# baldhat/yolov10-3D

Hardware: AMD Instinct MI355X
Metric: train_images_per_sec (higher is better)
Workload: dtype bf16

## Files before the change

### include/y3d.h

```cpp
#ifndef Y3D_H
#define Y3D_H
#include <stdint.h>

#ifdef __cplusplus
extern "C" {
#endif

enum { Y3D_F32 = 0, Y3D_BF16 = 1 };
enum { Y3D_OK = 0, Y3D_ERR_INVALID = -1, Y3D_ERR_HIP = -2 };

const char* y3d_last_error(void);
int y3d_abi_version(void);
int y3d_device_info(char* name, int name_len, int* compute_units, int* lds_bytes, int* clock_khz);

int y3d_pack_weight_fwd(int dtype, const float* w_oihw, void* out, int Cout, int Cin_g, int Cin_g_pad, int kh, int kw, void* stream);
int y3d_pack_weight_dgrad(int dtype, const float* w_oihw, void* out, int Cout, int Cin_g, int groups, int kh, int kw, void* stream);
int y3d_mt_pack_weights(int dtype, const int64_t* desc, const int* chunk_tensor, const int* chunk_off, int nchunks, int chunk, void* stream);
int y3d_mt_fp8w_quantize(const int64_t* desc, const int* row_begin, int ntensors, int nrows, void* stream);
int y3d_fp8w_dequantize(const uint8_t* codes, const float* scale, float* w, int rows, int K, void* stream);
int y3d_fp8_quantize_act(const void* x, int64_t xsw, int64_t M, int C, uint8_t* q, uint8_t* s, void* stream);
int y3d_fp8_pack_weight_fwd(const uint8_t* codes, const float* scale, int rows, int Cg, uint8_t* wq, uint8_t* ws, void* stream);
int y3d_conv3x3_fp8_ok(int B, int H, int W, int Cin, int Cout, int groups);
int y3d_conv3x3_fp8_stat_rows(int B, int H, int W);
int y3d_fp8_scale_pitch(int C);
// ... 2 lines not shown
int y3d_conv_kpad(int dtype, int k_total);
int y3d_conv_stat_blocks(int B, int Ho, int Wo);
int y3d_conv2d_stat_rows(int dtype, int B, int H, int W, int Cin, int Cout, int groups, int kh, int kw, int stride, int pad);
int y3d_conv2d_fwd(int dtype, const void* x, int64_t xsb, int64_t xsh, int64_t xsw, int B, int H, int W, int Cin,
                   const void* w_packed, const float* bias, void* y, int64_t ysw, int Ho, int Wo, int Cout, int groups,
                   int kh, int kw, int stride, int pad, float* stat_partials, void* stream);
int y3d_conv2d_fwd_affine(int dtype, const void* x, int64_t xsb, int64_t xsh, int64_t xsw, int B, int H, int W, int Cin,
                          const void* w_packed, const float* scale, const float* shift, int act, void* y, int64_t ysw, int Ho, int Wo,
                          int Cout, int groups, int kh, int kw, int stride, int pad, void* stream);
int y3d_conv2d_fwd_affine_res_ok(int dtype, int B, int H, int W, int Cin, int Cout, int groups, int kh, int kw, int stride, int pad);
int y3d_conv2d_fwd_affine_res(int dtype, const void* x, int64_t xsb, int64_t xsh, int64_t xsw, int B, int H, int W, int Cin,
                              const void* w_packed, const float* scale, const float* shift, int act, const void* res, int64_t rsw, void* y,
                              int64_t ysw, int Ho, int Wo, int Cout, int groups, int kh, int kw, int stride, int pad, void* stream);
int y3d_conv2d_bwd_data(int dtype, const void* dy, int64_t dsb, int64_t dsh, int64_t dsw, int B, int Ho, int Wo, int Cout,
                        const void* w_packed_dgrad, void* dx, int64_t xsw, int H, int W, int Cin, int groups, int kh, int kw,
                        int stride, int pad, void* stream);
int y3d_conv2d_wgrad_splits(int dtype, int B, int Ho, int Wo, int Cout, int Cin_g, int groups, int kh, int kw);
int y3d_conv2d_wgrad_plan(int dtype, int B, int H, int W, int Cin, int Cout, int groups, int kh, int kw, int stride, int pad);
int y3d_set_tile_kernels(int enable);
int y3d_set_stream1x1(int enable);
int y3d_get_stream1x1(void);
int y3d_get_tile_kernels(void);
int y3d_set_bn_wide_slabs(int enable);
int y3d_conv2d_bwd_weight(int dtype, const void* x, int64_t xsb, int64_t xsh, int64_t xsw, int B, int H, int W, int Cin,
                          int Cin_real, const void* dy, int64_t dsw, int Ho, int Wo, int Cout, int groups, int kh, int kw,
                          int stride, int pad, float* slab, int nsplit, float* grad_oihw, int accumulate, void* stream);

int y3d_dw_blocks(int64_t M);
int y3d_dw_wgrad_blocks(int64_t M);
int y3d_dw_pack_weight(const float* w_oihw, float* out_taps_c, int C, int kh, int kw, void* stream);
int y3d_dwconv2d_fwd(int dtype, const void* x, int64_t xsb, int64_t xsh, int64_t xsw, int B, int H, int W, int C,
                     const float* w_packed, void* y, int64_t ysw, int Ho, int Wo, int kh, int kw, int stride, int pad,
                     float* stat_partials, void* stream);
int y3d_dwconv2d_fwd_affine(int dtype, const void* x, int64_t xsb, int64_t xsh, int64_t xsw, int B, int H, int W, int C,
                            const float* w_packed, const float* scale, const float* shift, int act, int res_mode, const void* res, int64_t rsw,
                            void* z, int64_t zsw, int Ho, int Wo, int kh, int kw, int stride, int pad, void* stream);
int y3d_dwconv2d_bwd_data(int dtype, const void* dy, int64_t dsb, int64_t dsh, int64_t dsw, int B, int Ho, int Wo, int C,
                          const float* w_packed, void* dx, int64_t xsw, int H, int W, int kh, int kw, int stride, int pad,
                          void* stream);
int y3d_dwconv2d_bwd_weight(int dtype, const void* x, int64_t xsb, int64_t xsh, int64_t xsw, int B, int H, int W, int C,
                            const void* dy, int64_t dsw, int Ho, int Wo, int kh, int kw, int stride, int pad, float* slab,
                            float* grad_oihw, int accumulate, void* stream);

int y3d_bn_finalize(const float* partials, int nblk, int C, int64_t count, const float* gamma, const float* beta, float eps,
                    float momentum, float* running_mean, float* running_var, float* mean, float* invstd, float* scale,
                    float* shift, void* stream);
// ... 138 lines not shown
```

### yolov10-3d_amd/_lib.py

```python
from __future__ import annotations

import ctypes
import os
import re

_HERE = os.path.dirname(os.path.abspath(__file__))
LIB_PATH = os.path.join(_HERE, "liby3d_hip.so")
HEADER = os.path.join(os.path.dirname(_HERE), "include", "y3d.h")

F32, BF16 = 0, 1

_CT = {"int": ctypes.c_int, "int64_t": ctypes.c_int64, "float": ctypes.c_float, "double": ctypes.c_double}


class Y3DError(RuntimeError):
    pass


def parse_header(path: str = HEADER):
    src = open(path).read()
    src = re.sub(r"/\*.*?\*/", " ", src, flags=re.S)
    protos = {}
    for m in re.finditer(r"(const\s+char\s*\*|int)\s+(y3d_\w+)\s*\(([^;{]*?)\)\s*;", src, flags=re.S):
        ret, name, args = m.group(1), m.group(2), m.group(3).strip()
        argtypes = []
        if args and args != "void":
            for a in args.split(","):
                a = a.strip()
                if "*" in a:
                    argtypes.append(ctypes.c_void_p)
                else:
                    toks = a.split()
                    t = toks[1] if toks[0] == "const" else toks[0]
                    argtypes.append(_CT[t])
        protos[name] = (ctypes.c_char_p if "char" in ret else ctypes.c_int, argtypes)
    return protos


_PLAIN_INT = {"abi_version", "conv_kpad", "conv_stat_blocks", "conv2d_stat_rows", "conv2d_wgrad_splits", "conv2d_wgrad_plan", "set_tile_kernels", "set_stream1x1", "set_bn_wide_slabs", "get_stream1x1", "get_tile_kernels", "dw_blocks", "dw_wgrad_blocks", "bn_bwd_blocks", "proj_blocks", "proj_group_blocks", "proj_group_bn_bwd_blocks", "proj_group_bwd_weight_bn_mfma_blocks", "tal3d_scratch_floats", "v10_postprocess_scratch_floats", "conv2d_fwd_affine_res_ok", "stem_conv_train_rows", "conv3x3_fp8_ok", "conv3x3_fp8_stat_rows", "fp8_scale_pitch"}


class _Lib:
    def __init__(self):
        if not os.path.exists(LIB_PATH):
            raise Y3DError(
                f"{LIB_PATH} not found: build it with `python yolov10-3d_amd/csrc/build.py` "
                "(or __graft_entry__.build()). There is no CPU / PyTorch fallback for the HIP path.")
        self._dll = ctypes.CDLL(LIB_PATH)
        self.protos = parse_header()
        for name, (ret, argtypes) in self.protos.items():
            fn = getattr(self._dll, name)
            fn.restype = ret
            fn.argtypes = argtypes

    def last_error(self) -> str:
        return (self._dll.y3d_last_error() or b"").decode()

    def __getattr__(self, name):
        if name.startswith("_"):
            raise AttributeError(name)
        fn = getattr(self._dll, "y3d_" + name)
        ret = self.protos["y3d_" + name][0]
        if ret is not ctypes.c_int or name in _PLAIN_INT:
            setattr(self, name, fn)
            return fn

        def call(*a):
            rc = fn(*a)
            if rc != 0:
                raise Y3DError(f"y3d_{name} failed ({rc}): {self.last_error()}")
            return rc

        setattr(self, name, call)
        return call


# ... 9 lines not shown
```

### yolov10-3d_amd/csrc/conv3x3_flat.hip

```cpp
#include "common.h"

namespace {


struct WFP {
  const bf16_t* x;
  const bf16_t* w;
  bf16_t* y;
  float* part;
  const float* scale;
  const float* shift;
  int act;
  long xsb, xsh, xsw, ysw;
  int B, H, W;
  int Cg, Cn, G;
  int Ktot;
  int ntf, ntc;
  int flip;
  unsigned xbytes, wbytes;
  int HP, WP, IMG;
  int HPIX;
  float inv_img, inv_wp;
};

template <int N> __device__ __forceinline__ void wvm() { asm volatile("s_waitcnt vmcnt(%0)" ::"n"(N) : "memory"); }

__device__ __forceinline__ void wvm_n(int n) {
  switch (n) {
    case 0: wvm<0>(); break; case 1: wvm<1>(); break; case 2: wvm<2>(); break; case 3: wvm<3>(); break;
    case 4: wvm<4>(); break; case 5: wvm<5>(); break; case 6: wvm<6>(); break; case 7: wvm<7>(); break;
    case 8: wvm<8>(); break; case 9: wvm<9>(); break; case 10: wvm<10>(); break; case 11: wvm<11>(); break;
    case 12: wvm<12>(); break; case 13: wvm<13>(); break; case 14: wvm<14>(); break; case 15: wvm<15>(); break;
    case 16: wvm<16>(); break; case 17: wvm<17>(); break; case 18: wvm<18>(); break; case 19: wvm<19>(); break;
    case 20: wvm<20>(); break; case 21: wvm<21>(); break; case 22: wvm<22>(); break; case 23: wvm<23>(); break;
    case 24: wvm<24>(); break; case 25: wvm<25>(); break; case 26: wvm<26>(); break; case 27: wvm<27>(); break;
    case 28: wvm<28>(); break;
    default: wvm<0>(); break;
  }
}

__device__ __forceinline__ bf16x8_t ldf(const char* p) { return __builtin_bit_cast(bf16x8_t, *(const uint4*)p); }
__device__ __forceinline__ void lgk0() { asm volatile("s_waitcnt lgkmcnt(0)" ::: "memory"); }

template <int NHB, int EPI, bool HROLE>
__device__ __forceinline__ void flat_body(const WFP& p) {
  constexpr int HD = NHB - 1;
  constexpr int RD = 4, D = 3;
  constexpr int WB = 8192;
  extern __shared__ __attribute__((aligned(16))) char smem[];
  const int HBYTES = p.HPIX * 64;
  const int NI = p.HPIX >> 4;
  const int HR = NI >> 2;
  char* sH = smem;
  char* sW = smem + NHB * HBYTES;
  float* red = (float*)(sW + RD * WB);

  const int tid = threadIdx.x, lane = tid & 63, wave = __builtin_amdgcn_readfirstlane(tid >> 6);
  const int wc = wave & 1, wp = wave >> 1;
  const int wl = wave & 3;
  const int nslab = (p.Cg + 31) >> 5;

  const int ntiles = p.G * p.ntf * p.ntc;
  int tile, tile_end, tile_step;
  {
    const int xcd = blockIdx.x & 7, slot = blockIdx.x >> 3;
    tile_step = gridDim.x >> 3;
    const int lo = (int)((long)ntiles * xcd / 8);
    tile_end = (int)((long)ntiles * (xcd + 1) / 8);
    tile = lo + slot;
  }
  if (tile >= tile_end) return;

  struct TileC { int g, f0, c0, tf, live; };
  auto decode = [&](int t, bool live) {
    TileC c;
    int tc = t % p.ntc; t /= p.ntc;
    c.tf = t % p.ntf; c.g = t / p.ntf;
    c.f0 = c.tf * 512; c.c0 = tc * 128; c.live = live;
    return c;
  };

  constexpr unsigned OOB = 0xfffffff0u;
  const __amdgpu_buffer_rsrc_t rx = __builtin_amdgcn_make_buffer_rsrc((void*)p.x, 0, (int)p.xbytes, 0x00020000);
  const __amdgpu_buffer_rsrc_t rw = __builtin_amdgcn_make_buffer_rsrc((void*)p.w, 0, (int)p.wbytes, 0x00020000);
  const int xsw2 = (int)p.xsw * 2, xsh2 = (int)p.xsh * 2, xsb2 = (int)p.xsb * 2;
  const int lj0 = lane >> 2;
  const int pc0 = ((lane & 3) << 4) ^ ((lj0 & 4) << 3);
  const int a64 = 64 / p.WP, c64 = 64 - a64 * p.WP;
  int hb = 0, hy = 0, hx = 0;
  auto issue_h = [&](const TileC& c, int slab, int bufo, int rd) {
    if (rd == 0) {
      int lj = lj0;
      asm volatile("" : "+v"(lj));
      const int fs = c.f0 - (p.WP + 1) + 16 * wl + lj + p.IMG;
      int q = (int)((float)fs * p.inv_img);
      int r = fs - q * p.IMG;
      if (r < 0) { r += p.IMG; --q; }
      if (r >= p.IMG) { r -= p.IMG; ++q; }
      int y = (int)((float)r * p.inv_wp);
      int x = r - y * p.WP;
      if (x < 0) { x += p.WP; --y; }
// ... 9 lines not shown
    const unsigned off = (unsigned)(hb * xsb2 + (hy - 1) * xsh2 + __mul24(hx - 1, xsw2) + (c.g * p.Cg + slab * 32) * 2 + pc0);
    char* dst = sH + bufo + (rd * 4 + wl) * 1024;
    __builtin_amdgcn_raw_ptr_buffer_load_lds(rx, (__attribute__((address_space(3))) void*)dst, 16, ok ? off : OOB, 0, 0, 0);
  };
  const int ltid = tid & 255;
  int wrel0, wrel1, wch;
  {
    const int n0 = ltid >> 2, s = ltid & 3;
    wch = (s ^ (((n0 >> 4) & 1) << 1)) << 3;
    wrel0 = (n0 * p.Ktot + wch) * 2;
    wrel1 = ((n0 + 64) * p.Ktot + wch) * 2;
  }
  auto issue_w = [&](const TileC& c, int slab, int tap, int slot, int rd) {
    const unsigned base = (unsigned)((c.g * p.Cn + c.c0) * p.Ktot + (p.flip ? 8 - tap : tap) * p.Cg + slab * 32) * 2u;
    const int n = rd * 64 + (ltid >> 2);
    const bool ok = (c.live != 0) & (c.c0 + n < p.Cn) & (wch < p.Cg - slab * 32);
    __builtin_amdgcn_raw_ptr_buffer_load_lds(rw, (__attribute__((address_space(3))) void*)(sW + slot * WB + (rd * 256 + wl * 64) * 16), 16,
                                             ok ? base + (unsigned)(rd ? wrel1 : wrel0) : OOB, 0, 0, 0);
  };

  const int lp = lane & 15, lq = lane >> 4;
  const int arow = wc * 64 + (lp >> 2) * 8 + (lp & 3);
  const int ao = arow * 64 + ((lq ^ (((arow >> 4) & 1) << 1)) << 4);
  const int pb0 = wp * 128 + lp;
  bf16x8_t fa[4], fb[4];
  int bo;
  auto set_tap = [&](int tap) {
    const int r = tap / 3, q = tap - r * 3;
    const int pb = pb0 + r * p.WP + q;
    bo = (pb << 6) + ((lq ^ ((pb >> 1) & 2)) << 4);
  };
  auto load_b = [&](int bufo, int half) {
    const char* hbp = sH + bufo + bo;
#pragma unroll
    for (int i = 0; i < 4; ++i) fb[i] = ldf(hbp + (half * 4 + i) * 1024);
  };
  auto load_a = [&](int slot) {
#pragma unroll
    for (int ct = 0; ct < 4; ++ct) fa[ct] = ldf(sW + slot * WB + ao + (ct >> 1) * 2048 + (ct & 1) * 256);
  };

  TileC cur = decode(tile, true);
  TileC nx = decode(tile + tile_step < tile_end ? tile + tile_step : tile, tile + tile_step < tile_end);
  if (HROLE) {
#pragma unroll 1
    for (int h = 0; h < HD; ++h)
#pragma unroll 1
      for (int rd = 0; rd < HR; ++rd) issue_h(cur, h, h * HBYTES, rd);
    wvm_n((HD - 1) * HR);
  } else {
#pragma unroll
    for (int t = 0; t < D; ++t) { issue_w(cur, 0, t, t, 0); issue_w(cur, 0, t, t, 1); }
    wvm<2 * (D - 1)>();
  }
  __builtin_amdgcn_s_barrier();

  int gs = 0;
  int ho_cur = 0, ho_nxt = HBYTES, ho_tgt = (NHB - 1) * HBYTES;
  int tolerate = 0;
#pragma unroll 1
  for (; tile < tile_end; tile += tile_step) {
    f32x4_t acc[4][8];
#pragma unroll
    for (int a = 0; a < 4; ++a)
#pragma unroll
      for (int c = 0; c < 8; ++c) acc[a][c] = (f32x4_t){0.f, 0.f, 0.f, 0.f};

    if (!HROLE) __builtin_amdgcn_s_barrier();

#pragma unroll 1
    for (int k = 0; k < nslab; ++k, ++gs) {
      const bool last = k == nslab - 1;
      const int kr = gs & 3;
      const int hb_cur = ho_cur, hb_nxt = ho_nxt, hb_tgt = ho_tgt;
      if (NHB == 3) { ho_cur = hb_nxt; ho_nxt = hb_tgt; ho_tgt = hb_cur; } else { ho_cur = hb_nxt; ho_nxt = hb_cur; ho_tgt = hb_cur; }
      const bool hin = k + HD < nslab;
      const int hs = hin ? k + HD : k + HD - nslab;
      const TileC htile = hin ? cur : nx;
      const TileC wtile = last ? nx : cur;
      const int wslab = last ? 0 : k + 1;
#pragma unroll
      for (int t = 0; t < 9; ++t) {
        const int t2 = t + D;
        set_tap(t);
        load_a((kr + t) & 3);
        load_b(hb_cur, 0);
        __builtin_amdgcn_sched_barrier(0);
        if (HROLE) {
          if (2 * t < HR) issue_h(htile, hs, hb_tgt, 2 * t);
        } else {
          if (t2 < 9) issue_w(cur, k, t2, (kr + t2) & 3, 0); else issue_w(wtile, wslab, t2 - 9, (kr + t2) & 3, 0);
        }
        __builtin_amdgcn_sched_barrier(0);
        lgk0();
        __builtin_amdgcn_sched_barrier(0);
        __builtin_amdgcn_s_barrier();
        __builtin_amdgcn_s_setprio(1);
#pragma unroll
        for (int ct = 0; ct < 4; ++ct)
#pragma unroll
          for (int i = 0; i < 4; ++i) acc[ct][i] = __builtin_amdgcn_mfma_f32_16x16x32_bf16(fa[ct], fb[i], acc[ct][i], 0, 0, 0);
        __builtin_amdgcn_s_setprio(0);
        __builtin_amdgcn_sched_barrier(0);
        __builtin_amdgcn_s_barrier();
        load_b(hb_cur, 1);
        __builtin_amdgcn_sched_barrier(0);
        if (HROLE) {
          if (2 * t + 1 < HR) issue_h(htile, hs, hb_tgt, 2 * t + 1);
          if (t == 8) { if (NHB == 3) wvm_n(HR); else wvm<0>(); }
        } else {
          if (t2 < 9) issue_w(cur, k, t2, (kr + t2) & 3, 1); else issue_w(wtile, wslab, t2 - 9, (kr + t2) & 3, 1);
          if (k == 0 && t < 2) wvm_n(2 * (D - 1) + tolerate);
          else wvm<2 * (D - 1)>();
        }
        __builtin_amdgcn_sched_barrier(0);
        lgk0();
        __builtin_amdgcn_sched_barrier(0);
        __builtin_amdgcn_s_barrier();
        __builtin_amdgcn_s_setprio(1);
#pragma unroll
        for (int ct = 0; ct < 4; ++ct)
#pragma unroll
          for (int i = 0; i < 4; ++i) acc[ct][4 + i] = __builtin_amdgcn_mfma_f32_16x16x32_bf16(fa[ct], fb[i], acc[ct][4 + i], 0, 0, 0);
        __builtin_amdgcn_s_setprio(0);
        __builtin_amdgcn_sched_barrier(0);
        __builtin_amdgcn_s_barrier();
      }
    }
    if (HROLE) __builtin_amdgcn_s_barrier();

    int el = ltid;
    asm volatile("" : "+v"(el));
    const int e_lp = el & 15, e_lq = (el >> 4) & 3;
    const int e_tid = (HROLE ? 0 : 256) + el;
    const int cl0 = wc * 64 + e_lq * 8;
    const int a16 = 16 / p.WP, c16 = 16 - a16 * p.WP;
    int eb, ey, ex;
    {
      const int f = cur.f0 + wp * 128 + e_lp;
      int q = (int)((float)f * p.inv_img);
      int r = f - q * p.IMG;
      if (r < 0) { r += p.IMG; --q; }
      if (r >= p.IMG) { r -= p.IMG; ++q; }
      int y = (int)((float)r * p.inv_wp);
      int x = r - y * p.WP;
      if (x < 0) { x += p.WP; --y; }
      if (x >= p.WP) { x -= p.WP; ++y; }
      eb = q; ey = y; ex = x;
    }
    bool cok[2];
    typedef float f2_t __attribute__((ext_vector_type(2)));
    typedef __bf16 b2_t __attribute__((ext_vector_type(2)));
    f2_t s2[2][4], q2[2][4];
    float sv[2][8], hv[2][8];
#pragma unroll
    for (int h = 0; h < 2; ++h) {
      cok[h] = cur.c0 + cl0 + h * 32 < p.Cn;
#pragma unroll
      for (int i = 0; i < 4; ++i) { s2[h][i] = (f2_t){0.f, 0.f}; q2[h][i] = (f2_t){0.f, 0.f}; }
      if (EPI == 1) {
#pragma unroll
        for (int i = 0; i < 8; ++i) {
          sv[h][i] = cok[h] ? p.scale[cur.g * p.Cn + cur.c0 + cl0 + h * 32 + i] : 1.f;
          hv[h][i] = cok[h] ? p.shift[cur.g * p.Cn + cur.c0 + cl0 + h * 32 + i] : 0.f;
        }
      }
    }
    int issued = 0;
#pragma unroll
    for (int pt = 0; pt < 8; ++pt) {
      const bool pok = ((unsigned)eb < (unsigned)p.B) & ((unsigned)(ey - 1) < (unsigned)p.H) & ((unsigned)(ex - 1) < (unsigned)p.W);
      const unsigned keep = pok ? 0xffffffffu : 0u;
      bf16_t* dst = p.y + (((long)eb * p.H + (ey - 1)) * p.W + (ex - 1)) * p.ysw + (long)cur.g * p.Cn + cur.c0 + cl0;
#pragma unroll
      for (int h = 0; h < 2; ++h) {
        if (EPI == 0) {
          unsigned pk[4];
#pragma unroll
          for (int c2 = 0; c2 < 2; ++c2)
#pragma unroll
            for (int jj = 0; jj < 2; ++jj) {
              const f2_t a = {acc[2 * h + c2][pt][2 * jj], acc[2 * h + c2][pt][2 * jj + 1]};
              const unsigned u = __builtin_bit_cast(unsigned, __builtin_convertvector(a, b2_t)) & keep;
              pk[c2 * 2 + jj] = u;
              const f2_t r = {__uint_as_float(u << 16), __uint_as_float(u & 0xffff0000u)};
              s2[h][c2 * 2 + jj] += r;
              q2[h][c2 * 2 + jj] = __builtin_elementwise_fma(r, r, q2[h][c2 * 2 + jj]);
            }
          if (pok && cok[h]) *(uint4*)(dst + h * 32) = make_uint4(pk[0], pk[1], pk[2], pk[3]);
        } else {
          float v[8];
#pragma unroll
          for (int c2 = 0; c2 < 2; ++c2)
// ... 27 lines not shown
      lgk0();
      __builtin_amdgcn_s_barrier();
      if (e_tid < 128) {
        const int ch = e_tid;
        if (cur.c0 + ch < p.Cn) {
          float s = 0.f, q = 0.f;
#pragma unroll
          for (int w = 0; w < 4; ++w) { s += red[(w * 128 + ch) * 2]; q += red[(w * 128 + ch) * 2 + 1]; }
          float* dst = p.part + ((long)cur.tf * (p.G * p.Cn) + cur.g * p.Cn + cur.c0 + ch) * 2;
          *(float2*)dst = make_float2(s, q);
        }
      }
    }
    tolerate = __builtin_amdgcn_readfirstlane(issued);
    cur = nx;
    {
      const int t2 = tile + 2 * tile_step;
      nx = decode(t2 < tile_end ? t2 : tile, t2 < tile_end);
    }
  }
  wvm<0>();
}

template <int NHB, int EPI>
__global__ __launch_bounds__(512, 1) void conv3x3_flat_kernel(WFP p) {
  if (__builtin_amdgcn_readfirstlane(threadIdx.x >> 6) < 4) flat_body<NHB, EPI, true>(p);
  else flat_body<NHB, EPI, false>(p);
}

int flat_cu_count() {
  static int n = 0;
  if (!n) {
    int dev = 0;
    hipDeviceProp_t pr;
    if (hipGetDevice(&dev) == hipSuccess && hipGetDeviceProperties(&pr, dev) == hipSuccess) n = pr.multiProcessorCount;
    if (n <= 0) n = 256;
  }
  return n;
}

template <int NHB, int EPI>
int launch_flat(const WFP& p, hipStream_t st) {
  size_t sm = (size_t)NHB * p.HPIX * 64 + 4 * 8192 + 4 * 128 * 2 * 4;
  static bool attr_set = false;
  if (!attr_set) {
    (void)hipFuncSetAttribute((const void*)conv3x3_flat_kernel<NHB, EPI>, hipFuncAttributeMaxDynamicSharedMemorySize, 160 * 1024);
    attr_set = true;
  }
  long ntiles = (long)p.G * p.ntf * p.ntc;
  long nwg = (long)flat_cu_count() / 8 * 8;
  if (nwg < 8) nwg = 8;
  while (nwg > 8 && nwg / 8 > (ntiles + 7) / 8) nwg -= 8;
  hipLaunchKernelGGL((conv3x3_flat_kernel<NHB, EPI>), dim3((unsigned)nwg), dim3(512), sm, st, p);
  Y3D_LAUNCH_CHECK();
  return Y3D_OK;
}

}

static int flat_hpix(int W) { return (512 + 2 * (W + 3) + 63) / 64 * 64; }

int y3d_conv3x3_flat_tiles(int B, int H, int W) { return cdiv((long)B * (H + 2) * (W + 2), 512); }

int y3d_conv3x3_flat_ok(int B, int H, int W, int Cg, int Cn, int G) {
  if (Cg % 8 != 0 || Cg < 40 || Cn % 16 != 0 || W < 8 || W > 126 || H < 8) return 0;
  if ((size_t)2 * flat_hpix(W) * 64 + 4 * 8192 + 4096 > 160 * 1024) return 0;
  if ((long)B * (H + 2) * (W + 2) >= (1L << 23)) return 0;
  return 1;
}

int y3d_conv3x3_flat_launch(const void* x, long xsb, long xsh, long xsw, int B, int H, int W, int Cg, int Cn, int G, const void* w, int Ktot, void* y,
                            long ysw, float* part, int flip, const float* scale, const float* shift, int act, void* stream) {
  WFP p;
  p.x = (const bf16_t*)x; p.w = (const bf16_t*)w; p.y = (bf16_t*)y; p.part = part; p.scale = scale; p.shift = shift; p.act = act;
  p.xsb = xsb; p.xsh = xsh; p.xsw = xsw; p.ysw = ysw;
  p.B = B; p.H = H; p.W = W; p.Cg = Cg; p.Cn = Cn; p.G = G; p.Ktot = Ktot;
  p.HP = H + 2; p.WP = W + 2; p.IMG = p.HP * p.WP; p.HPIX = flat_hpix(W);
  p.inv_img = 1.0f / (float)p.IMG; p.inv_wp = 1.0f / (float)p.WP;
  p.ntf = y3d_conv3x3_flat_tiles(B, H, W); p.ntc = cdiv(Cn, 128); p.flip = flip;
  const unsigned long xb = ((unsigned long)(B - 1) * xsb + (unsigned long)(H - 1) * xsh + (unsigned long)(W - 1) * xsw + (unsigned long)G * Cg) * 2;
  const unsigned long wb = (unsigned long)G * Cn * Ktot * 2;
  Y3D_CHECK(xb < 0xfffffff0ul && wb < 0xfffffff0ul, "conv3x3_flat: operand larger than 4 GB");
  Y3D_CHECK(2 * xsw < (1L << 23) && Ktot < (1 << 22), "conv3x3_flat: pixel stride beyond the 24-bit address multiply");
  Y3D_CHECK(y3d_conv3x3_flat_ok(B, H, W, Cg, Cn, G), "conv3x3_flat: geometry not served");
  p.xbytes = (unsigned)xb; p.wbytes = (unsigned)wb;
  hipStream_t st = (hipStream_t)stream;
  const bool three = (size_t)3 * p.HPIX * 64 + 4 * 8192 + 4096 <= 160 * 1024;
  if (three) return scale ? launch_flat<3, 1>(p, st) : launch_flat<3, 0>(p, st);
  return scale ? launch_flat<2, 1>(p, st) : launch_flat<2, 0>(p, st);
}
```

### yolov10-3d_amd/csrc/conv3x3_tile.hip

```cpp
#include "common.h"
#include <cstdlib>
#include "conv_frag.h"

namespace {

__device__ uint4 y3d_zero_page[4];
#ifdef Y3D_PROBE_STAMP
__device__ unsigned long long y3d_probe_stamps[16384 * 4];
#define Y3D_STAMP(i) if (threadIdx.x == 0 && blockIdx.z * gridDim.x + blockIdx.x < 16384) y3d_probe_stamps[(blockIdx.z * gridDim.x + blockIdx.x) * 4 + (i)] = __builtin_amdgcn_s_memtime()
#else
#define Y3D_STAMP(i)
#endif

struct C3P {
  const void* x;
  const void* w;
  void* y;
  float* part;
  const float* scale;
  const float* shift;
  int act;
  long xsb, xsh, xsw, ysw;
  int B, H, W;
  int Cg, Cn, G;
// ... 242 lines not shown
  constexpr int RD = TH == 16 ? 4 : 2;
  size_t sm = 2 * (size_t)HCH * 16 + (size_t)RD * 16384;
  static bool attr_set = false;
  if (!attr_set) {
    (void)hipFuncSetAttribute((const void*)conv3x3_tile_kernel<T, TH, EPI>, hipFuncAttributeMaxDynamicSharedMemorySize, (int)sm);
    attr_set = true;
  }
  dim3 grid(p.B * p.nty * p.ntx * p.ntc, 1, p.G);
  hipLaunchKernelGGL((conv3x3_tile_kernel<T, TH, EPI>), grid, dim3(NT), sm, st, p);
  Y3D_LAUNCH_CHECK();
  return Y3D_OK;
}

template <typename T, int TH>
int launch_tile_epi(const C3P& p, hipStream_t st) {
  return p.scale ? launch_tile<T, TH, 1>(p, st) : launch_tile<T, TH, 0>(p, st);
}

}

int y3d_conv3x3_wide3_launch(int th, const void* x, long xsb, long xsh, long xsw, int B, int H, int W, int Cg, int Cn, int G, const void* w,
                             int Ktot, void* y, long ysw, float* part, int flip, const float* scale, const float* shift, int act, void* stream);

int y3d_conv3x3_flat_ok(int B, int H, int W, int Cg, int Cn, int G);
int y3d_conv3x3_flat_tiles(int B, int H, int W);
int y3d_conv3x3_flat_launch(const void* x, long xsb, long xsh, long xsw, int B, int H, int W, int Cg, int Cn, int G, const void* w, int Ktot, void* y,
                            long ysw, float* part, int flip, const float* scale, const float* shift, int act, void* stream);

static int v2_max_tiles() { return 129; }

int y3d_tile_height(int dtype, int B, int H, int W, int Cg, int Cn, int G, int kh, int kw, int stride, int pad) {
  int cse = 32;
  if (kh != 3 || kw != 3 || stride != 1 || pad != 1) return 0;
  if (dtype == Y3D_BF16 ? (Cg % 8 != 0 || Cg < 40 || (Cg < 64 && Cg % 32 != 0 && Cn <= 64)) : (Cg % cse != 0 || Cg < 64)) return 0;
  if (Cn % 16 != 0) return 0;
  if (W < 8) return 0;
  if (dtype == Y3D_BF16 && y3d_conv3x3_flat_ok(B, H, W, Cg, Cn, G)) {
    const int thr = H % 16 == 0 ? 16 : 8;
    const long rect = (long)cdiv(B, 32 / thr) * cdiv(H, thr) * cdiv(W, 16), flat = y3d_conv3x3_flat_tiles(B, H, W);
    if (flat * 104 < rect * 100 && flat * G * cdiv(Cn, 128) >= v2_max_tiles()) return -1;
  }
  if (H % 16 == 0) return 16;
  if (H % 8 == 0) return 8;
  if (dtype == Y3D_BF16 && H > 8 && (H % 8) >= 4 && (long)G * cdiv(B, 4) * cdiv(H, 8) * cdiv(W, 16) * cdiv(Cn, 128) >= v2_max_tiles()) return 8;
  return 0;
}

int y3d_conv3x3_tile_launch(int dtype, int th, const void* x, long xsb, long xsh, long xsw, int B, int H, int W, int Cg, int Cn, int G,
                            const void* w, int Ktot, void* y, long ysw, float* part, int flip, const float* scale, const float* shift, int act,
                            void* stream) {
  C3P p;
  p.x = x; p.w = w; p.y = y; p.part = part; p.scale = scale; p.shift = shift; p.act = act;
  p.xsb = xsb; p.xsh = xsh; p.xsw = xsw; p.ysw = ysw;
  p.B = B; p.H = H; p.W = W; p.Cg = Cg; p.Cn = Cn; p.G = G; p.Ktot = Ktot;
  p.ntx = cdiv(W, 16); p.nty = cdiv(H, th); p.ntc = cdiv(Cn, 128); p.flip = flip;
  hipStream_t st = (hipStream_t)stream;
  if (th < 0) return y3d_conv3x3_flat_launch(x, xsb, xsh, xsw, B, H, W, Cg, Cn, G, w, Ktot, y, ysw, part, flip, scale, shift, act, stream);
  if (dtype == Y3D_BF16) {
    const long wide_tiles = (long)G * cdiv(B, 32 / th) * p.nty * p.ntx * p.ntc;
    if (wide_tiles < v2_max_tiles() && Cg % 64 == 0 && H % th == 0)
      return th == 16 ? launch_tile_epi<bf16_t, 16>(p, st) : launch_tile_epi<bf16_t, 8>(p, st);
    return y3d_conv3x3_wide3_launch(th, x, xsb, xsh, xsw, B, H, W, Cg, Cn, G, w, Ktot, y, ysw, part, flip, scale, shift, act, stream);
  }
  return th == 16 ? launch_tile_epi<float, 16>(p, st) : launch_tile_epi<float, 8>(p, st);
}
```

### yolov10-3d_amd/csrc/conv_gemm.hip

```cpp
#include "common.h"
#include "conv_frag.h"
#include <cstdlib>

namespace {

struct ConvP {
  const void* x;
  const void* w;
  const float* bias;
  const float* scale;
  const float* shift;
  int act;
  void* y;
  float* part;
  long xsb, xsh, xsw;
  long ysw;
  int B, Hg, Wg;
  int Hq, Wq;
  int Cg, Cn, G;
  int kh, kw, stride, pad;
  int Ktot, Kpad;
  int M;
  int ntx, nty;
};
// ... 631 lines not shown
  if (bc == 128) {
    size_t sm = 2 * (128 + 128) * 128;
    hipLaunchKernelGGL((conv_gemm_kernel<T, 128, 128, 2, 2, MODE>), dim3(p.ntx * p.nty, ny, p.G), block, sm, st, p);
  } else if (bc == 64) {
    size_t sm = 2 * (128 + 64) * 128;
    hipLaunchKernelGGL((conv_gemm_kernel<T, 128, 64, 4, 1, MODE>), dim3(p.ntx * p.nty, ny, p.G), block, sm, st, p);
  } else {
    size_t sm = 2 * (128 + 32) * 128;
    hipLaunchKernelGGL((conv_gemm_kernel<T, 128, 32, 4, 1, MODE>), dim3(p.ntx * p.nty, ny, p.G), block, sm, st, p);
  }
  Y3D_LAUNCH_CHECK();
  return Y3D_OK;
}

template <typename T, bool DGRAD>
int launch_conv(ConvP p, hipStream_t st) {
  if (DGRAD && p.kh == 3 && p.kw == 3 && p.stride == 2 && p.pad == 1 && p.Cg % TT<T>::CE == 0) return launch_conv_mode<T, 2>(p, st);
  return launch_conv_mode<T, DGRAD ? 1 : 0>(p, st);
}

}

int y3d_tile_height(int dtype, int B, int H, int W, int Cg, int Cn, int G, int kh, int kw, int stride, int pad);
int y3d_conv3x3_flat_tiles(int B, int H, int W);
int y3d_conv3x3_tile_launch(int dtype, int th, const void* x, long xsb, long xsh, long xsw, int B, int H, int W, int Cg, int Cn, int G,
                            const void* w, int Ktot, void* y, long ysw, float* part, int flip, const float* scale, const float* shift, int act,
                            void* stream);

int y3d_wgrad_tile_height(int dtype, int H, int W, int Cg, int Cn, int kh, int kw, int stride, int pad);
int y3d_wgrad_tile_splits(int th, int B, int H, int W, int Cg, int Cn, int G);
int y3d_conv3x3_wgrad_tile_launch(int th, const void* x, long xsb, long xsh, long xsw, const void* dy, long dsw, int B, int H, int W, int Cg,
                                  int Cn, int G, float* slab, int nsplit, void* stream);

int y3d_conv1x1_stream_ok(int dtype, long M, int K, int N, long xsw, int G = 1);
int y3d_conv1x1_stream_launch(const void* x, long xsw, const void* w, int Kpad, const float* bias, const float* scale, const float* shift, int act,
                              void* y, long ysw, float* part, long M, int K, int N, int G, void* stream);
int y3d_wgrad1x1_stream_ok(int dtype, long M, int Cg, int Cn, long xsw, long dsw);
int y3d_wgrad1x1_stream_launch(const void* x, long xsw, const void* dy, long dsw, long M, int Cg, int Cn, float* slab, int nsplit, int chunk_px,
                               void* stream);
int y3d_conv3x3s2_dgrad_ok(int dtype, int B, int Ho, int Wo, int H, int W, int Cout, int Cin, long dsw, long xsw);
int y3d_conv3x3s2_dgrad_launch(const void* dy, long dsw, int B, int Ho, int Wo, int Cout, const void* w_packed_dgrad, int Kpad, void* dx, long xsw,
                               int H, int W, int Cin, void* stream);
int y3d_conv3x3_small_ok(int dtype, int B, int H, int W, int Cin, int Cout, int rows);
int y3d_conv3x3_small_launch(const void* x, long xsb, long xsh, long xsw, int B, int H, int W, int Cin, int Cout, const void* w, int Ktot, void* y,
                             long ysw, float* part, int rows, int flip, const float* scale, const float* shift, int act, const void* res, long rsw,
                             void* stream);
int y3d_conv3x3_small_rows(int B, int H, int W, int Cin, int Cout);
// ... 30 lines not shown
  if (kh == 3 && kw == 3 && stride == 1 && pad == 1 && groups == 1 && y3d_wgrad3x3_small_ok(dtype, B, H, W, Cin, Cout))
    return y3d_wgrad3x3_small_splits(B, H, W);
  int th = (g_tile_kernels && groups > 0) ? y3d_wgrad_tile_height(dtype, H, W, Cin / groups, Cout / groups, kh, kw, stride, pad) : 0;
  if (th) return y3d_wgrad_tile_splits(th, B, H, W, Cin / groups, Cout / groups, groups);
  int Ho = (H + 2 * pad - kh) / stride + 1, Wo = (W + 2 * pad - kw) / stride + 1;
  if (kh == 1 && kw == 1 && stride == 1 && pad == 0 && groups == 1 && y3d_wgrad1x1_stream_ok(dtype, (long)B * H * W, Cin, Cout, Cin, Cout)) {
    const int target = 256;
    const long tiles = (long)cdiv(Cin, Cin <= 64 ? 64 : 128) * cdiv(Cout, Cout <= 64 ? 64 : 128);
    long want = target / tiles, maxs = cdiv((long)B * H * W, 4 * 64);
    if (want > maxs) want = maxs;
    return (int)(want < 1 ? 1 : want);
  }
  return y3d_conv2d_wgrad_splits(dtype, B, Ho, Wo, Cout, Cin / groups, groups, kh, kw);
}

int y3d_conv2d_stat_rows(int dtype, int B, int H, int W, int Cin, int Cout, int groups, int kh, int kw, int stride, int pad) {
  if (kh == 1 && kw == 1 && stride == 1 && pad == 0 && groups >= 1 && y3d_conv1x1_stream_ok(dtype, (long)B * H * W, Cin / groups, Cout / groups, Cin, groups))
    return y3d_conv1x1_stream_rows((long)B * H * W, Cin / groups, Cout / groups, groups);
  if (kh == 3 && kw == 3 && stride == 1 && pad == 1 && groups == 1 && y3d_conv3x3_small_ok(dtype, B, H, W, Cin, Cout, 1))
    return y3d_conv3x3_small_rows(B, H, W, Cin, Cout);
  if (kh == 3 && kw == 3 && stride == 2 && pad == 1 && groups == 1 && y3d_conv3x3_small_s2_ok(dtype, B, H, W, Cin, Cout))
    return y3d_conv3x3_small_s2_rows(B, H, W, Cin, Cout);
  int th = (g_tile_kernels && groups > 0) ? y3d_tile_height(dtype, B, H, W, Cin / groups, Cout / groups, groups, kh, kw, stride, pad) : 0;
  if (th < 0) return y3d_conv3x3_flat_tiles(B, H, W);
  if (th) return B * cdiv(H, th) * cdiv(W, 16);
  int Ho = (H + 2 * pad - kh) / stride + 1, Wo = (W + 2 * pad - kw) / stride + 1;
  return cdiv((long)B * Ho * Wo, 128);
}

int y3d_conv_kpad(int dtype, int k_total) {
  int ce = dtype == Y3D_BF16 ? 8 : 4;
  return cdiv(k_total, ce) * ce;
}

int y3d_pack_weight_fwd(int dtype, const float* w_oihw, void* out, int Cout, int Cin_g, int Cin_g_pad, int kh, int kw, void* stream) {
  int ce = dtype == Y3D_BF16 ? 8 : 4;
  Y3D_CHECK(Cin_g_pad >= Cin_g && Cin_g_pad % ce == 0, "pack_weight_fwd: Cin_g_pad=%d must be a multiple of %d", Cin_g_pad, ce);
  int taps = kh * kw, Kpad = taps * Cin_g_pad;
  long n = (long)Cout * Kpad;
  hipStream_t st = (hipStream_t)stream;
  if (dtype == Y3D_BF16)
    hipLaunchKernelGGL(pack_w_fwd_kernel<bf16_t>, dim3(cdiv(n, 256)), dim3(256), 0, st, w_oihw, (bf16_t*)out, Cout, Cin_g, Cin_g_pad, taps, Kpad);
  else
    hipLaunchKernelGGL(pack_w_fwd_kernel<float>, dim3(cdiv(n, 256)), dim3(256), 0, st, w_oihw, (float*)out, Cout, Cin_g, Cin_g_pad, taps, Kpad);
  Y3D_LAUNCH_CHECK();
  return Y3D_OK;
}
// ... 230 lines not shown
```

Measured before the change: 1425.

## Add 256-position flat conv3x3 tile variant with cost-model tiling selection

```diff
diff --git a/include/y3d.h b/include/y3d.h
--- a/include/y3d.h
+++ b/include/y3d.h
@@ -48,6 +48,8 @@
 int y3d_get_stream1x1(void);
 int y3d_get_tile_kernels(void);
 int y3d_set_bn_wide_slabs(int enable);
+int y3d_set_flat256(int mode);
+int y3d_conv3x3_tiling(int dtype, int B, int H, int W, int Cg, int Cn, int G);
 int y3d_conv2d_bwd_weight(int dtype, const void* x, int64_t xsb, int64_t xsh, int64_t xsw, int B, int H, int W, int Cin,
                           int Cin_real, const void* dy, int64_t dsw, int Ho, int Wo, int Cout, int groups, int kh, int kw,
                           int stride, int pad, float* slab, int nsplit, float* grad_oihw, int accumulate, void* stream);
diff --git a/yolov10-3d_amd/_lib.py b/yolov10-3d_amd/_lib.py
--- a/yolov10-3d_amd/_lib.py
+++ b/yolov10-3d_amd/_lib.py
@@ -37,7 +37,7 @@
     return protos
 
 
-_PLAIN_INT = {"abi_version", "conv_kpad", "conv_stat_blocks", "conv2d_stat_rows", "conv2d_wgrad_splits", "conv2d_wgrad_plan", "set_tile_kernels", "set_stream1x1", "set_bn_wide_slabs", "get_stream1x1", "get_tile_kernels", "dw_blocks", "dw_wgrad_blocks", "bn_bwd_blocks", "proj_blocks", "proj_group_blocks", "proj_group_bn_bwd_blocks", "proj_group_bwd_weight_bn_mfma_blocks", "tal3d_scratch_floats", "v10_postprocess_scratch_floats", "conv2d_fwd_affine_res_ok", "stem_conv_train_rows", "conv3x3_fp8_ok", "conv3x3_fp8_stat_rows", "fp8_scale_pitch"}
+_PLAIN_INT = {"abi_version", "conv_kpad", "conv_stat_blocks", "conv2d_stat_rows", "conv2d_wgrad_splits", "conv2d_wgrad_plan", "set_tile_kernels", "set_stream1x1", "set_bn_wide_slabs", "set_flat256", "conv3x3_tiling", "get_stream1x1", "get_tile_kernels", "dw_blocks", "dw_wgrad_blocks", "bn_bwd_blocks", "proj_blocks", "proj_group_blocks", "proj_group_bn_bwd_blocks", "proj_group_bwd_weight_bn_mfma_blocks", "tal3d_scratch_floats", "v10_postprocess_scratch_floats", "conv2d_fwd_affine_res_ok", "stem_conv_train_rows", "conv3x3_fp8_ok", "conv3x3_fp8_stat_rows", "fp8_scale_pitch"}
 
 
 class _Lib:
@@ -52,6 +52,9 @@
             fn = getattr(self._dll, name)
             fn.restype = ret
             fn.argtypes = argtypes
+        flat256 = os.environ.get("Y3D_FLAT256")
+        if flat256 in ("0", "1", "2"):
+            self._dll.y3d_set_flat256(int(flat256))
 
     def last_error(self) -> str:
         return (self._dll.y3d_last_error() or b"").decode()
diff --git a/yolov10-3d_amd/csrc/conv3x3_flat.hip b/yolov10-3d_amd/csrc/conv3x3_flat.hip
--- a/yolov10-3d_amd/csrc/conv3x3_flat.hip
+++ b/yolov10-3d_amd/csrc/conv3x3_flat.hip
@@ -42,8 +42,10 @@
 __device__ __forceinline__ bf16x8_t ldf(const char* p) { return __builtin_bit_cast(bf16x8_t, *(const uint4*)p); }
 __device__ __forceinline__ void lgk0() { asm volatile("s_waitcnt lgkmcnt(0)" ::: "memory"); }
 
-template <int NHB, int EPI, bool HROLE>
+template <int NP, int NHB, int EPI, bool HROLE>
 __device__ __forceinline__ void flat_body(const WFP& p) {
+  static_assert(NP == 512 || NP == 256, "flat tile of 512 or 256 positions");
+  constexpr int PW = NP / 4, NC = PW / 16, NH = NC / 2;
   constexpr int HD = NHB - 1;
   constexpr int RD = 4, D = 3;
   constexpr int WB = 8192;
@@ -76,7 +78,7 @@
     TileC c;
     int tc = t % p.ntc; t /= p.ntc;
     c.tf = t % p.ntf; c.g = t / p.ntf;
-    c.f0 = c.tf * 512; c.c0 = tc * 128; c.live = live;
+    c.f0 = c.tf * NP; c.c0 = tc * 128; c.live = live;
     return c;
   };
 
@@ -132,8 +134,8 @@
   const int lp = lane & 15, lq = lane >> 4;
   const int arow = wc * 64 + (lp >> 2) * 8 + (lp & 3);
   const int ao = arow * 64 + ((lq ^ (((arow >> 4) & 1) << 1)) << 4);
-  const int pb0 = wp * 128 + lp;
-  bf16x8_t fa[4], fb[4];
+  const int pb0 = wp * PW + lp;
+  bf16x8_t fa[4], fb[NH];
   int bo;
   auto set_tap = [&](int tap) {
     const int r = tap / 3, q = tap - r * 3;
@@ -143,7 +145,7 @@
   auto load_b = [&](int bufo, int half) {
     const char* hbp = sH + bufo + bo;
 #pragma unroll
-    for (int i = 0; i < 4; ++i) fb[i] = ldf(hbp + (half * 4 + i) * 1024);
+    for (int i = 0; i < NH; ++i) fb[i] = ldf(hbp + (half * NH + i) * 1024);
   };
   auto load_a = [&](int slot) {
 #pragma unroll
@@ -170,11 +172,11 @@
   int tolerate = 0;
 #pragma unroll 1
   for (; tile < tile_end; tile += tile_step) {
-    f32x4_t acc[4][8];
+    f32x4_t acc[4][NC];
 #pragma unroll
     for (int a = 0; a < 4; ++a)
 #pragma unroll
-      for (int c = 0; c < 8; ++c) acc[a][c] = (f32x4_t){0.f, 0.f, 0.f, 0.f};
+      for (int c = 0; c < NC; ++c) acc[a][c] = (f32x4_t){0.f, 0.f, 0.f, 0.f};
 
     if (!HROLE) __builtin_amdgcn_s_barrier();
 
@@ -209,7 +211,7 @@
 #pragma unroll
         for (int ct = 0; ct < 4; ++ct)
 #pragma unroll
-          for (int i = 0; i < 4; ++i) acc[ct][i] = __builtin_amdgcn_mfma_f32_16x16x32_bf16(fa[ct], fb[i], acc[ct][i], 0, 0, 0);
+          for (int i = 0; i < NH; ++i) acc[ct][i] = __builtin_amdgcn_mfma_f32_16x16x32_bf16(fa[ct], fb[i], acc[ct][i], 0, 0, 0);
         __builtin_amdgcn_s_setprio(0);
         __builtin_amdgcn_sched_barrier(0);
         __builtin_amdgcn_s_barrier();
@@ -231,7 +233,7 @@
 #pragma unroll
         for (int ct = 0; ct < 4; ++ct)
 #pragma unroll
-          for (int i = 0; i < 4; ++i) acc[ct][4 + i] = __builtin_amdgcn_mfma_f32_16x16x32_bf16(fa[ct], fb[i], acc[ct][4 + i], 0, 0, 0);
+          for (int i = 0; i < NH; ++i) acc[ct][NH + i] = __builtin_amdgcn_mfma_f32_16x16x32_bf16(fa[ct], fb[i], acc[ct][NH + i], 0, 0, 0);
         __builtin_amdgcn_s_setprio(0);
         __builtin_amdgcn_sched_barrier(0);
         __builtin_amdgcn_s_barrier();
@@ -247,7 +249,7 @@
     const int a16 = 16 / p.WP, c16 = 16 - a16 * p.WP;
     int eb, ey, ex;
     {
-      const int f = cur.f0 + wp * 128 + e_lp;
+      const int f = cur.f0 + wp * PW + e_lp;
       int q = (int)((float)f * p.inv_img);
       int r = f - q * p.IMG;
       if (r < 0) { r += p.IMG; --q; }
@@ -278,7 +280,7 @@
     }
     int issued = 0;
 #pragma unroll
-    for (int pt = 0; pt < 8; ++pt) {
+    for (int pt = 0; pt < NC; ++pt) {
       const bool pok = ((unsigned)eb < (unsigned)p.B) & ((unsigned)(ey - 1) < (unsigned)p.H) & ((unsigned)(ex - 1) < (unsigned)p.W);
       const unsigned keep = pok ? 0xffffffffu : 0u;
       bf16_t* dst = p.y + (((long)eb * p.H + (ey - 1)) * p.W + (ex - 1)) * p.ysw + (long)cur.g * p.Cn + cur.c0 + cl0;
@@ -352,10 +354,10 @@
   wvm<0>();
 }
 
-template <int NHB, int EPI>
+template <int NP, int NHB, int EPI>
 __global__ __launch_bounds__(512, 1) void conv3x3_flat_kernel(WFP p) {
-  if (__builtin_amdgcn_readfirstlane(threadIdx.x >> 6) < 4) flat_body<NHB, EPI, true>(p);
-  else flat_body<NHB, EPI, false>(p);
+  if (__builtin_amdgcn_readfirstlane(threadIdx.x >> 6) < 4) flat_body<NP, NHB, EPI, true>(p);
+  else flat_body<NP, NHB, EPI, false>(p);
 }
 
 int flat_cu_count() {
@@ -369,53 +371,58 @@
   return n;
 }
 
-template <int NHB, int EPI>
+template <int NP, int NHB, int EPI>
 int launch_flat(const WFP& p, hipStream_t st) {
   size_t sm = (size_t)NHB * p.HPIX * 64 + 4 * 8192 + 4 * 128 * 2 * 4;
   static bool attr_set = false;
   if (!attr_set) {
-    (void)hipFuncSetAttribute((const void*)conv3x3_flat_kernel<NHB, EPI>, hipFuncAttributeMaxDynamicSharedMemorySize, 160 * 1024);
+    (void)hipFuncSetAttribute((const void*)conv3x3_flat_kernel<NP, NHB, EPI>, hipFuncAttributeMaxDynamicSharedMemorySize, 160 * 1024);
     attr_set = true;
   }
   long ntiles = (long)p.G * p.ntf * p.ntc;
   long nwg = (long)flat_cu_count() / 8 * 8;
   if (nwg < 8) nwg = 8;
   while (nwg > 8 && nwg / 8 > (ntiles + 7) / 8) nwg -= 8;
-  hipLaunchKernelGGL((conv3x3_flat_kernel<NHB, EPI>), dim3((unsigned)nwg), dim3(512), sm, st, p);
+  hipLaunchKernelGGL((conv3x3_flat_kernel<NP, NHB, EPI>), dim3((unsigned)nwg), dim3(512), sm, st, p);
   Y3D_LAUNCH_CHECK();
   return Y3D_OK;
 }
 
 }
 
-static int flat_hpix(int W) { return (512 + 2 * (W + 3) + 63) / 64 * 64; }
-
-int y3d_conv3x3_flat_tiles(int B, int H, int W) { return cdiv((long)B * (H + 2) * (W + 2), 512); }
-
-int y3d_conv3x3_flat_ok(int B, int H, int W, int Cg, int Cn, int G) {
+static int flat_hpix(int W, int np) { return (np + 2 * (W + 3) + 63) / 64 * 64; }
+
+int y3d_conv3x3_flat_tiles(int B, int H, int W, int np) { return cdiv((long)B * (H + 2) * (W + 2), np); }
+
+int y3d_conv3x3_flat_ok(int B, int H, int W, int Cg, int Cn, int G, int np) {
+  if (np != 512 && np != 256) return 0;
   if (Cg % 8 != 0 || Cg < 40 || Cn % 16 != 0 || W < 8 || W > 126 || H < 8) return 0;
-  if ((size_t)2 * flat_hpix(W) * 64 + 4 * 8192 + 4096 > 160 * 1024) return 0;
+  if ((size_t)2 * flat_hpix(W, np) * 64 + 4 * 8192 + 4096 > 160 * 1024) return 0;
   if ((long)B * (H + 2) * (W + 2) >= (1L << 23)) return 0;
   return 1;
 }
 
 int y3d_conv3x3_flat_launch(const void* x, long xsb, long xsh, long xsw, int B, int H, int W, int Cg, int Cn, int G, const void* w, int Ktot, void* y,
-                            long ysw, float* part, int flip, const float* scale, const float* shift, int act, void* stream) {
+                            long ysw, float* part, int flip, const float* scale, const float* shift, int act, int np, void* stream) {
   WFP p;
   p.x = (const bf16_t*)x; p.w = (const bf16_t*)w; p.y = (bf16_t*)y; p.part = part; p.scale = scale; p.shift = shift; p.act = act;
   p.xsb = xsb; p.xsh = xsh; p.xsw = xsw; p.ysw = ysw;
   p.B = B; p.H = H; p.W = W; p.Cg = Cg; p.Cn = Cn; p.G = G; p.Ktot = Ktot;
-  p.HP = H + 2; p.WP = W + 2; p.IMG = p.HP * p.WP; p.HPIX = flat_hpix(W);
+  p.HP = H + 2; p.WP = W + 2; p.IMG = p.HP * p.WP; p.HPIX = flat_hpix(W, np);
   p.inv_img = 1.0f / (float)p.IMG; p.inv_wp = 1.0f / (float)p.WP;
-  p.ntf = y3d_conv3x3_flat_tiles(B, H, W); p.ntc = cdiv(Cn, 128); p.flip = flip;
+  p.ntf = y3d_conv3x3_flat_tiles(B, H, W, np); p.ntc = cdiv(Cn, 128); p.flip = flip;
   const unsigned long xb = ((unsigned long)(B - 1) * xsb + (unsigned long)(H - 1) * xsh + (unsigned long)(W - 1) * xsw + (unsigned long)G * Cg) * 2;
   const unsigned long wb = (unsigned long)G * Cn * Ktot * 2;
   Y3D_CHECK(xb < 0xfffffff0ul && wb < 0xfffffff0ul, "conv3x3_flat: operand larger than 4 GB");
   Y3D_CHECK(2 * xsw < (1L << 23) && Ktot < (1 << 22), "conv3x3_flat: pixel stride beyond the 24-bit address multiply");
-  Y3D_CHECK(y3d_conv3x3_flat_ok(B, H, W, Cg, Cn, G), "conv3x3_flat: geometry not served");
+  Y3D_CHECK(y3d_conv3x3_flat_ok(B, H, W, Cg, Cn, G, np), "conv3x3_flat: geometry not served (%d-position tiles)", np);
   p.xbytes = (unsigned)xb; p.wbytes = (unsigned)wb;
   hipStream_t st = (hipStream_t)stream;
   const bool three = (size_t)3 * p.HPIX * 64 + 4 * 8192 + 4096 <= 160 * 1024;
-  if (three) return scale ? launch_flat<3, 1>(p, st) : launch_flat<3, 0>(p, st);
-  return scale ? launch_flat<2, 1>(p, st) : launch_flat<2, 0>(p, st);
-}
+  if (np == 256) {
+    Y3D_CHECK(three, "conv3x3_flat: 256-position halo buffers do not fit");
+    return scale ? launch_flat<256, 3, 1>(p, st) : launch_flat<256, 3, 0>(p, st);
+  }
+  if (three) return scale ? launch_flat<512, 3, 1>(p, st) : launch_flat<512, 3, 0>(p, st);
+  return scale ? launch_flat<512, 2, 1>(p, st) : launch_flat<512, 2, 0>(p, st);
+}
diff --git a/yolov10-3d_amd/csrc/conv3x3_tile.hip b/yolov10-3d_amd/csrc/conv3x3_tile.hip
--- a/yolov10-3d_amd/csrc/conv3x3_tile.hip
+++ b/yolov10-3d_amd/csrc/conv3x3_tile.hip
@@ -288,12 +288,64 @@
 int y3d_conv3x3_wide3_launch(int th, const void* x, long xsb, long xsh, long xsw, int B, int H, int W, int Cg, int Cn, int G, const void* w,
                              int Ktot, void* y, long ysw, float* part, int flip, const float* scale, const float* shift, int act, void* stream);
 
-int y3d_conv3x3_flat_ok(int B, int H, int W, int Cg, int Cn, int G);
-int y3d_conv3x3_flat_tiles(int B, int H, int W);
+int y3d_conv3x3_flat_ok(int B, int H, int W, int Cg, int Cn, int G, int np);
+int y3d_conv3x3_flat_tiles(int B, int H, int W, int np);
 int y3d_conv3x3_flat_launch(const void* x, long xsb, long xsh, long xsw, int B, int H, int W, int Cg, int Cn, int G, const void* w, int Ktot, void* y,
-                            long ysw, float* part, int flip, const float* scale, const float* shift, int act, void* stream);
+                            long ysw, float* part, int flip, const float* scale, const float* shift, int act, int np, void* stream);
 
 static int v2_max_tiles() { return 129; }
+
+static int g_flat256 = 1;
+
+static int rect_height(int dtype, int B, int H, int W, int Cn, int G) {
+  if (H % 16 == 0) return 16;
+  if (H % 8 == 0) return 8;
+  if (dtype == Y3D_BF16 && H > 8 && (H % 8) >= 4 && (long)G * cdiv(B, 4) * cdiv(H, 8) * cdiv(W, 16) * cdiv(Cn, 128) >= v2_max_tiles()) return 8;
+  return 0;
+}
+
+static bool tile_kernel_takes(int th, int B, int H, int W, int Cg, int Cn, int G) {
+  const long wide_tiles = (long)G * cdiv(B, 32 / th) * cdiv(H, th) * cdiv(W, 16) * cdiv(Cn, 128);
+  return wide_tiles < v2_max_tiles() && Cg % 64 == 0 && H % th == 0;
+}
+
+struct TilingCost { long ns_per_k, k0; };
+static const TilingCost kCostWide = {23, 100}, kCostFlat512 = {23, 100}, kCostFlat256 = {13, 540};
+static long persistent_rounds(long tiles) { return cdiv(cdiv(tiles, 8), 32); }
+static long round_ns(const TilingCost& c, long K) { return c.ns_per_k * (K + c.k0); }
+
+static int flat_cost_pick(int round4, int B, int H, int W, int Cg, int Cn, int G) {
+  const int rect = rect_height(Y3D_BF16, B, H, W, Cn, G);
+  const long ntc = (long)G * cdiv(Cn, 128);
+  const long K = 9L * 32 * cdiv(Cg, 32);
+  long best = -1, work = 0;
+  int code = round4;
+  auto consider = [&](long c, long w, int th) {
+    if (best < 0 || c < best || (c == best && w < work)) { best = c; work = w; code = th; }
+  };
+  if (rect > 0 && !tile_kernel_takes(rect, B, H, W, Cg, Cn, G)) {
+    const long t = cdiv(B, 32 / rect) * cdiv(H, rect) * cdiv(W, 16) * ntc;
+    consider(persistent_rounds(t) * round_ns(kCostWide, K), t * 512, rect);
+  }
+  if (y3d_conv3x3_flat_ok(B, H, W, Cg, Cn, G, 512)) {
+    const long t = y3d_conv3x3_flat_tiles(B, H, W, 512) * ntc;
+    consider(persistent_rounds(t) * round_ns(kCostFlat512, K), t * 512, -1);
+  }
+  if (y3d_conv3x3_flat_ok(B, H, W, Cg, Cn, G, 256)) {
+    const long t = y3d_conv3x3_flat_tiles(B, H, W, 256) * ntc;
+    consider(persistent_rounds(t) * round_ns(kCostFlat256, K), t * 256, -2);
+  }
+  return code;
+}
+
+static int round4_height(int dtype, int B, int H, int W, int Cg, int Cn, int G) {
+  if (dtype == Y3D_BF16 && y3d_conv3x3_flat_ok(B, H, W, Cg, Cn, G, 512)) {
+    const int thr = H % 16 == 0 ? 16 : 8;
+    const long rect = (long)cdiv(B, 32 / thr) * cdiv(H, thr) * cdiv(W, 16), flat = y3d_conv3x3_flat_tiles(B, H, W, 512);
+    if (flat * 104 < rect * 100 && flat * G * cdiv(Cn, 128) >= v2_max_tiles()) return -1;
+  }
+  return rect_height(dtype, B, H, W, Cn, G);
+}
 
 int y3d_tile_height(int dtype, int B, int H, int W, int Cg, int Cn, int G, int kh, int kw, int stride, int pad) {
   int cse = 32;
@@ -301,15 +353,30 @@
   if (dtype == Y3D_BF16 ? (Cg % 8 != 0 || Cg < 40 || (Cg < 64 && Cg % 32 != 0 && Cn <= 64)) : (Cg % cse != 0 || Cg < 64)) return 0;
   if (Cn % 16 != 0) return 0;
   if (W < 8) return 0;
-  if (dtype == Y3D_BF16 && y3d_conv3x3_flat_ok(B, H, W, Cg, Cn, G)) {
-    const int thr = H % 16 == 0 ? 16 : 8;
-    const long rect = (long)cdiv(B, 32 / thr) * cdiv(H, thr) * cdiv(W, 16), flat = y3d_conv3x3_flat_tiles(B, H, W);
-    if (flat * 104 < rect * 100 && flat * G * cdiv(Cn, 128) >= v2_max_tiles()) return -1;
-  }
-  if (H % 16 == 0) return 16;
-  if (H % 8 == 0) return 8;
-  if (dtype == Y3D_BF16 && H > 8 && (H % 8) >= 4 && (long)G * cdiv(B, 4) * cdiv(H, 8) * cdiv(W, 16) * cdiv(Cn, 128) >= v2_max_tiles()) return 8;
-  return 0;
+  if (dtype == Y3D_BF16 && g_flat256 == 2 && y3d_conv3x3_flat_ok(B, H, W, Cg, Cn, G, 256)) return -2;
+  const int round4 = round4_height(dtype, B, H, W, Cg, Cn, G);
+  if (dtype == Y3D_BF16 && g_flat256 == 1 && (round4 < 0 || (round4 > 0 && !tile_kernel_takes(round4, B, H, W, Cg, Cn, G))))
+    return flat_cost_pick(round4, B, H, W, Cg, Cn, G);
+  return round4;
+}
+
+extern "C" {
+
+int y3d_set_flat256(int mode) {
+  const int old = g_flat256;
+  g_flat256 = mode == 0 ? 0 : (mode == 2 ? 2 : 1);
+  return old;
+}
+
+int y3d_conv3x3_tiling(int dtype, int B, int H, int W, int Cg, int Cn, int G) {
+  const int th = y3d_tile_height(dtype, B, H, W, Cg, Cn, G, 3, 3, 1, 1);
+  if (th == -2) return 6;
+  if (th == -1) return 5;
+  if (th == 0) return 0;
+  if (dtype == Y3D_BF16 && !tile_kernel_takes(th, B, H, W, Cg, Cn, G)) return th == 16 ? 4 : 3;
+  return th == 16 ? 2 : 1;
+}
+
 }
 
 int y3d_conv3x3_tile_launch(int dtype, int th, const void* x, long xsb, long xsh, long xsw, int B, int H, int W, int Cg, int Cn, int G,
@@ -321,10 +388,10 @@
   p.B = B; p.H = H; p.W = W; p.Cg = Cg; p.Cn = Cn; p.G = G; p.Ktot = Ktot;
   p.ntx = cdiv(W, 16); p.nty = cdiv(H, th); p.ntc = cdiv(Cn, 128); p.flip = flip;
   hipStream_t st = (hipStream_t)stream;
-  if (th < 0) return y3d_conv3x3_flat_launch(x, xsb, xsh, xsw, B, H, W, Cg, Cn, G, w, Ktot, y, ysw, part, flip, scale, shift, act, stream);
+  if (th < 0)
+    return y3d_conv3x3_flat_launch(x, xsb, xsh, xsw, B, H, W, Cg, Cn, G, w, Ktot, y, ysw, part, flip, scale, shift, act, th == -2 ? 256 : 512, stream);
   if (dtype == Y3D_BF16) {
-    const long wide_tiles = (long)G * cdiv(B, 32 / th) * p.nty * p.ntx * p.ntc;
-    if (wide_tiles < v2_max_tiles() && Cg % 64 == 0 && H % th == 0)
+    if (tile_kernel_takes(th, B, H, W, Cg, Cn, G))
       return th == 16 ? launch_tile_epi<bf16_t, 16>(p, st) : launch_tile_epi<bf16_t, 8>(p, st);
     return y3d_conv3x3_wide3_launch(th, x, xsb, xsh, xsw, B, H, W, Cg, Cn, G, w, Ktot, y, ysw, part, flip, scale, shift, act, stream);
   }
diff --git a/yolov10-3d_amd/csrc/conv_gemm.hip b/yolov10-3d_amd/csrc/conv_gemm.hip
--- a/yolov10-3d_amd/csrc/conv_gemm.hip
+++ b/yolov10-3d_amd/csrc/conv_gemm.hip
@@ -677,7 +677,7 @@
 }
 
 int y3d_tile_height(int dtype, int B, int H, int W, int Cg, int Cn, int G, int kh, int kw, int stride, int pad);
-int y3d_conv3x3_flat_tiles(int B, int H, int W);
+int y3d_conv3x3_flat_tiles(int B, int H, int W, int np);
 int y3d_conv3x3_tile_launch(int dtype, int th, const void* x, long xsb, long xsh, long xsw, int B, int H, int W, int Cg, int Cn, int G,
                             const void* w, int Ktot, void* y, long ysw, float* part, int flip, const float* scale, const float* shift, int act,
                             void* stream);
@@ -754,7 +754,7 @@
   if (kh == 3 && kw == 3 && stride == 2 && pad == 1 && groups == 1 && y3d_conv3x3_small_s2_ok(dtype, B, H, W, Cin, Cout))
     return y3d_conv3x3_small_s2_rows(B, H, W, Cin, Cout);
   int th = (g_tile_kernels && groups > 0) ? y3d_tile_height(dtype, B, H, W, Cin / groups, Cout / groups, groups, kh, kw, stride, pad) : 0;
-  if (th < 0) return y3d_conv3x3_flat_tiles(B, H, W);
+  if (th < 0) return y3d_conv3x3_flat_tiles(B, H, W, th == -2 ? 256 : 512);
   if (th) return B * cdiv(H, th) * cdiv(W, 16);
   int Ho = (H + 2 * pad - kh) / stride + 1, Wo = (W + 2 * pad - kw) / stride + 1;
   return cdiv((long)B * Ho * Wo, 128);
```

Result: no change. 1429, median of 6 (+0.3%).
